# BAMresearch/PGDrome

Hardware: AMD Instinct MI355X
Metric: PGD fixed-point iters/sec + SpMV HBM GB/s, 256^3 P1 space x 1D param (higher is better)
Workload: dtype f64

## Files before the change

### include/pgd_amd.h

```cpp
#ifndef PGD_AMD_H
#define PGD_AMD_H

#include <stdint.h>

#ifdef __cplusplus
extern "C" {
#endif

typedef int64_t pgd_handle;

enum {
    PGD_OK = 0,
    PGD_ERR_INVALID = -1,
    PGD_ERR_HIP = -2,
    PGD_ERR_NOMEM = -3,
    PGD_ERR_LIMIT = -4,
    PGD_ERR_SINGULAR = -5,
    PGD_ERR_NODEVICE = -6,
    PGD_ERR_TIMEOUT = -7,
    PGD_ERR_PEER = -8
};

enum {
    PGD_ATOM_MASS = 0,
// ... 168 lines not shown
                   double threshold, double *sample_stats, pgd_handle env_min, pgd_handle env_max, pgd_handle exceed,
                   pgd_handle fields);

int pgd_cell_gradient(pgd_handle ctx, pgd_handle mesh, pgd_handle u, const double *L, int q, pgd_handle scale_or_0,
                      pgd_handle out);

int pgd_eval_batch_norm(pgd_handle ctx, const pgd_handle *modes, int k, int q, const double *coefs, int64_t s, int want,
                        double threshold, double *sample_stats, pgd_handle env_min, pgd_handle env_max, pgd_handle exceed,
                        pgd_handle fields);
int pgd_eval_batch_grad(pgd_handle ctx, pgd_handle mesh, const pgd_handle *modes, int k, const double *L, int q,
                        pgd_handle scale_or_0, const double *coefs, int64_t s, int want, double threshold, double *sample_stats,
                        pgd_handle env_min, pgd_handle env_max, pgd_handle exceed, pgd_handle fields);
int pgd_eval_norm_last_shape(pgd_handle ctx, int *rows, int *staged);

enum {
    PGD_TUNE_PCG_SCALAR_S = 56,
    PGD_TUNE_PCG_FOLD_MARCH = 55,
    PGD_TUNE_BLOCK_STORAGE = 54,
    PGD_TUNE_PCG_RECOMPUTE_Q = 53,
    PGD_TUNE_EVAL_SAMPLE_CHUNK = 52,
    PGD_TUNE_EVAL_GRID_MAX = 51,
    PGD_TUNE_EVAL_VARIANT = 50,
    PGD_TUNE_PUSH_IN_UPDATE = 49,
    PGD_TUNE_STENCIL_ROWS = 48,
    PGD_TUNE_DIA_MARCH3 = 47,
    PGD_TUNE_SHARD_ONE_MARCH = 46,
    PGD_TUNE_HALO_OVERLAP_MIN_ROWS = 45,
    PGD_TUNE_COMM_SELF_PERIODIC = 44,
    PGD_TUNE_PCG_DERIVE_SCALED = 43,
    PGD_TUNE_MG_MARCH_MIN = 42,
// ... 33 lines not shown
    PGD_TUNE_SPMV_VARIANT = 13,
    PGD_TUNE_SPMV_ZCHUNK = 6,
    PGD_TUNE_SPMV_SYM = 3,
    PGD_TUNE_SPMV_DICT = 2
};
int pgd_tune(pgd_handle ctx, int knob, int64_t value);

int pgd_prof_enable(pgd_handle ctx, int on);
int pgd_prof_read(pgd_handle ctx, int64_t *launches, double *seconds, double *alg_bytes);
int pgd_prof_read_own(pgd_handle ctx, double *own_bytes);
int pgd_prof_read_update(pgd_handle ctx, int64_t *launches, double *seconds, double *bytes);
int pgd_prof_read_dropped(pgd_handle ctx, int64_t *dropped);
int pgd_prof_event_overhead(pgd_handle ctx, double *seconds);
int pgd_kernel_counts(pgd_handle ctx, int64_t *out, int n);
int pgd_pcg_recompute_counts(pgd_handle ctx, int64_t *updates);
int pgd_classify_counts(pgd_handle ctx, int64_t *full, int64_t *cached);
int pgd_mg_counts(pgd_handle ctx, int64_t *solves, int64_t *fallbacks);
int pgd_vmg_counts(pgd_handle ctx, int64_t *solves, int64_t *fallbacks, int64_t *levels);
int pgd_vmg_times(pgd_handle ctx, double *setup_ms, int64_t *march_passes);
int pgd_cmg_counts(pgd_handle ctx, int64_t *solves, int64_t *fallbacks, int64_t *levels);
int pgd_cmg_times(pgd_handle ctx, double *setup_ms, int64_t *march_passes);
int pgd_mg_slab_setup(pgd_handle ctx, pgd_handle A, int nz_global, int z_first, int64_t own0, int64_t own1,
                      int64_t *n_coarse, int *applies);
int pgd_mg_slab_fix_start(pgd_handle ctx, pgd_handle A, pgd_handle b, pgd_handle x, int64_t own0, int64_t own1);
int pgd_mg_slab_down(pgd_handle ctx, pgd_handle r, pgd_handle t);
int pgd_mg_slab_restrict(pgd_handle ctx, pgd_handle t, pgd_handle b1);
int pgd_mg_coarse(pgd_handle ctx, pgd_handle b1, pgd_handle x1);
int pgd_mg_slab_up(pgd_handle ctx, pgd_handle r, pgd_handle x1, pgd_handle t, pgd_handle z, int slot, double *dot);
int pgd_calib_stream(pgd_handle ctx, pgd_handle vec, int bytes_per_lane, int store);
int pgd_timer_start(pgd_handle ctx);
// ... 7 lines not shown
```

### pgdrome_amd/_lib.py

```python
from __future__ import annotations

import ctypes as C
from pathlib import Path

import numpy as np

LIB_PATH = Path(__file__).resolve().parent / "lib" / "libpgd_amd.so"

H = C.c_int64
I64 = C.c_int64
I32 = C.c_int32
F64 = C.c_double
PD = C.POINTER(C.c_double)
PI32 = C.POINTER(C.c_int32)
PI64 = C.POINTER(C.c_int64)
PH = C.POINTER(C.c_int64)
VP = C.c_void_p

PU8 = C.POINTER(C.c_uint8)
HALO_FN = C.CFUNCTYPE(C.c_int, VP, H, I64, I64, I64, I64)
ALLREDUCE_FN = C.CFUNCTYPE(C.c_int, VP, C.c_int, C.c_int)

SIGNATURES = {
    "pgd_ctx_create": (C.c_int, [C.c_int, VP, PH]),
# ... 95 lines not shown
    "pgd_comm_push": (C.c_int, [H, C.c_int, C.POINTER(C.c_int)]),
    "pgd_comm_allreduce_attach": (C.c_int, [H, PU8, C.POINTER(C.c_int)]),
    "pgd_comm_allreduce_direct": (C.c_int, [H, C.c_int, C.POINTER(C.c_int)]),
    "pgd_pcg_solve_sharded": (C.c_int, [H, H, H, H, I64, I64, I64, I64, F64, F64, C.c_int, C.POINTER(C.c_int), PD]),
    "pgd_op_symmetrize": (C.c_int, [H, H, C.POINTER(C.c_int)]),
    "pgd_op_classify": (C.c_int, [H, H, C.POINTER(C.c_int)]),
    "pgd_tune": (C.c_int, [H, C.c_int, I64]),
    "pgd_prof_enable": (C.c_int, [H, C.c_int]),
    "pgd_prof_read": (C.c_int, [H, PI64, PD, PD]),
    "pgd_prof_read_own": (C.c_int, [H, PD]),
    "pgd_prof_read_update": (C.c_int, [H, PI64, PD, PD]),
    "pgd_prof_read_dropped": (C.c_int, [H, PI64]),
    "pgd_prof_event_overhead": (C.c_int, [H, PD]),
    "pgd_kernel_counts": (C.c_int, [H, PI64, C.c_int]),
    "pgd_pcg_recompute_counts": (C.c_int, [H, PI64]),
    "pgd_classify_counts": (C.c_int, [H, PI64, PI64]),
    "pgd_mg_counts": (C.c_int, [H, PI64, PI64]),
    "pgd_vmg_counts": (C.c_int, [H, PI64, PI64, PI64]),
    "pgd_vmg_times": (C.c_int, [H, C.POINTER(C.c_double), PI64]),
    "pgd_cmg_counts": (C.c_int, [H, PI64, PI64, PI64]),
    "pgd_cmg_times": (C.c_int, [H, C.POINTER(C.c_double), PI64]),
    "pgd_calib_stream": (C.c_int, [H, H, C.c_int, C.c_int]),
    "pgd_timer_start": (C.c_int, [H]),
    "pgd_timer_stop": (C.c_int, [H, PD]),
}

NSLOTS = 64
EVAL_STATS, EVAL_ENVELOPE, EVAL_EXCEED, EVAL_FIELDS = 1, 2, 4, 8
TUNE_EVAL_VARIANT, TUNE_EVAL_GRID_MAX, TUNE_EVAL_SAMPLE_CHUNK = 50, 51, 52
TUNE_BLOCK_STORAGE = 54
TUNE_PCG_FOLD_MARCH, TUNE_PCG_SCALAR_S = 55, 56
BLOCK_F32, BLOCK_F64, BLOCK_MAXK = 0, 1, 64


ERR_TIMEOUT, ERR_PEER = -7, -8


class PgdError(RuntimeError):
    def __init__(self, code, msg):
        super().__init__(f"libpgd_amd error {code}: {msg}")
        self.code = code


_lib = None


# ... 631 lines not shown
                    update_launches=un.value, update_seconds=us.value, update_bytes=ub.value, dropped_noop_samples=dr.value,
                    event_overhead=ov.value)

    KERNEL_FAMILIES = ("csr", "csr_dict", "sym_rows", "dia_rows", "dia_march", "multi", "diac_march", "stencil_march")

    def kernel_counts(self):
        out = (C.c_int64 * 8)()
        self._ck(self.lib.pgd_kernel_counts(self.h, out, 8))
        return {k: int(out[i]) for i, k in enumerate(self.KERNEL_FAMILIES)}

    def pcg_recompute_updates(self):
        n = I64()
        self._ck(self.lib.pgd_pcg_recompute_counts(self.h, C.byref(n)))
        return n.value

    def classify_counts(self):
        full, cached = I64(), I64()
        self._ck(self.lib.pgd_classify_counts(self.h, C.byref(full), C.byref(cached)))
        return {"full": full.value, "cached": cached.value}

    def precondition(self, multigrid):
        self.tune(40, 1 if multigrid else 0)
        return self.mg_stats()["solves"]

    def mg_stats(self):
        a, b = I64(), I64()
        self._ck(self.lib.pgd_mg_counts(self.h, C.byref(a), C.byref(b)))
        return {"solves": a.value, "fallbacks": b.value}

    def precondition_variable(self, on):
# ... 30 lines not shown
```

### pgdrome_amd/csrc/pgd_ctx.hip

```cpp
#include <algorithm>
#include <cstdarg>
#include <cstring>
#include <mutex>

#include "pgd_internal.h"

namespace pgd {

static std::mutex g_mu;
static std::vector<std::unique_ptr<Ctx>> g_ctx;
static std::string g_global_err;

Ctx *get_ctx(pgd_handle h) {
    std::lock_guard<std::mutex> lk(g_mu);
    if (h < 1 || h > (pgd_handle)g_ctx.size()) return nullptr;
    return g_ctx[h - 1].get();
}

int fail(Ctx *c, int code, const char *fmt, ...) {
    char buf[512];
    va_list ap;
    va_start(ap, fmt);
    vsnprintf(buf, sizeof buf, fmt, ap);
    va_end(ap);
// ... 424 lines not shown

int pgd_kernel_counts(pgd_handle h, int64_t *out, int n) {
    PGD_CTX(c, h);
    if (!out || n < 0) return fail(c, PGD_ERR_INVALID, "kernel_counts: invalid arguments");
    for (int k = 0; k < n; ++k) out[k] = k < 8 ? c->kcount[k] : 0;
    return PGD_OK;
}

int pgd_pcg_recompute_counts(pgd_handle h, int64_t *updates) {
    PGD_CTX(c, h);
    if (!updates) return fail(c, PGD_ERR_INVALID, "pcg_recompute_counts: invalid arguments");
    *updates = c->pcg_recompute_launches;
    return PGD_OK;
}

int pgd_timer_start(pgd_handle h) {
    PGD_CTX(c, h);
    for (auto &e : c->timer_ev)
        if (!e) PGD_HIP(c, hipEventCreate(&e));
    PGD_HIP(c, hipEventRecord(c->timer_ev[0], c->stream));
    return PGD_OK;
}

int pgd_timer_stop(pgd_handle h, double *seconds) {
    PGD_CTX(c, h);
    if (!c->timer_ev[0] || !c->timer_ev[1] || !seconds) return fail(c, PGD_ERR_INVALID, "timer_stop: no timer running");
    PGD_HIP(c, hipEventRecord(c->timer_ev[1], c->stream));
    PGD_HIP(c, hipEventSynchronize(c->timer_ev[1]));
    float ms = 0.f;
    PGD_HIP(c, hipEventElapsedTime(&ms, c->timer_ev[0], c->timer_ev[1]));
// ... 6 lines not shown
```

### pgdrome_amd/csrc/pgd_internal.h

```cpp
#pragma once

#include <hip/hip_runtime.h>

#include <chrono>
#include <cstdint>
#include <cstdio>
#include <map>
#include <memory>
#include <string>
#include <vector>

#include "../../include/pgd_amd.h"

namespace pgd {

constexpr int WAVE = 64;
constexpr int TPB = 256;
constexpr int MAX_VEC_BLOCKS = 2048;
constexpr int N_XCD = 8;
constexpr int DICT_MAXP = 256;
constexpr int DICT_DLEN = 32;
constexpr size_t PAD_BYTES = 256;

enum { S_PQ = 2, S_TOL2 = 5, S_DMIN = 7 , S_TMP = 8  };
// ... 191 lines not shown
    int num_cu = 256;
    int spmv_dict = 1;
    int spmv_rows = 64;
    int64_t spmv_grid_min_plane_bytes = 0;
    int spmv_zchunk_force = 0;
    int fault_iteration = -1;
    int fault_stage = 0;
    int fault_stall_ms = 0;
    int64_t pcg_small_ss_rows = (int64_t)1 << 22;
    int pcg_small_ss = 1;
    int pcg_stream_hints = 1;
    int pcg_lag_x = 1;
    int pcg_recompute_q = 1;
    int64_t pcg_recompute_launches = 0;
    int pcg_fold_march = 0;
    int pcg_scalar_s = 1;
    int asm_lattice = 1;
    int spmv_fetch_depth = 6;
    int spmv_zchunk_coded2 = 96;
    int spmv_zchunk_coded = 24;
    int pcg_exact_phase = 1;
    int pcg_fold_finish = 1;
    int atom_fast = 1;
    int lazy_csr = 1;
    uint64_t next_serial = 1;
    int pcg_precond = 0;
    struct Mg *mg = nullptr;
    struct Mg *mg_slab = nullptr;
    int64_t mg_solves = 0, mg_fallbacks = 0;
    struct Vmg *vmg = nullptr;
// ... 114 lines not shown
int vec_sqrt(Ctx *c, double *v, int64_t n);
int vec_div_mul(Ctx *c, double *x, const double *sc, int64_t n, int mul);
int ensure_vals(Ctx *c, const Mesh *m, Csr *a);
bool atom_fast_form(Ctx *c, const Mesh *m, Csr *a, int64_t r0, int64_t r1);
int dia_classify(Ctx *c, const Mesh *m, Csr *a, int zrange_lo = -1, int zrange_hi = -1);
bool stencil_row_range(const Ctx *c, const Mesh *m, const Csr *a, int64_t r0, int64_t r1);
bool stencil_whole_grid(const Ctx *c, const Mesh *m, const Csr *a);
struct StencilFold {
    const double *prod; int nprod;
    const double *vec_in; int nvec;
    int par;
};
int stencil_update_blocks(const Ctx *c, const Mesh *m);
int launch_stencil_update(Ctx *c, const Mesh *m, const Csr *a, const double *p_in, double *p_out, double *x, double *r, const double *s,
                          double *pairs, int lag, double s_free = 0.0, const StencilFold *fold = nullptr);
int launch_stencil_pass(Ctx *c, const uint8_t *cls, int ident, const double cst[8], int nx, int ny, int nz, int zm0, int zm1,
                        const double *x, const double *b, double *y, double w, int epi, bool dot, int *nparts, int z0 = 0, int z1 = -1);
bool mg_prepare(Ctx *c, const Mesh *m, const Csr *a);
int mg_fix_start(Ctx *c, const Csr *a, const double *b, double *x, int64_t n);
int mg_vcycle(Ctx *c, const double *r, bool dot, int *nparts, double *z_out = nullptr);
double *mg_result(Ctx *c);
void mg_release(Ctx *c);
struct Vmg;
bool vmg_prepare(Ctx *c, Vmg *&M, const Mesh *m, const Csr *a);
int vmg_fix_start(Ctx *c, Vmg *M, const double *sc, const double *b, double *x, int64_t n);
int vmg_vcycle(Ctx *c, Vmg *M, const double *r, bool dot, int *nparts, double *z_out, int64_t *marches);
double *vmg_result(Vmg *M);
void vmg_note_setup(Ctx *c);
void vmg_release(Ctx *c);
bool cmg_prepare(Ctx *c, const Mesh *m, const Mesh *base, const Csr *a);
// ... 113 lines not shown
```

### pgdrome_amd/csrc/pgd_pcg.hip

```cpp
#include "pgd_internal.h"

#include <cmath>

#include <cstring>

#include <algorithm>

namespace pgd {

constexpr int MAXT = 8;
constexpr int CHECK_EVERY = 16;
constexpr int PROF_EAGER_EVERY = 8;

struct CombineArgs {
    const double *in[MAXT];
    double coef[MAXT];
    int n;
};

__global__ __launch_bounds__(TPB) void k_combine(CombineArgs A, double *__restrict__ out, const int *__restrict__ cols,
                                                 const uint8_t *__restrict__ colmask, int64_t nnz) {
    for (int64_t k = (int64_t)blockIdx.x * TPB + threadIdx.x; k < nnz; k += (int64_t)gridDim.x * TPB) {
        double s = 0.0;
#pragma unroll
// ... 1244 lines not shown
}

struct PcgRun {
    static constexpr int S_INIT = 18, S_PAIR = 16;
    Ctx *c; const Mesh *m; Csr *o; const double *b; double *x; int64_t n;
    double *r, *z, *p, *q, *sc;
    double *part2 = nullptr, *part2b = nullptr;
    int gvec = 0, g2v = 0;
    PcgForm form = PGD_PCG_FORM_TEXTBOOK;
    PcgPrecond precond = PGD_PCG_PRECOND_JACOBI;
    bool scaled = false, lag_x = false;
    bool x_scaled = false;
    bool virt = false;
    double s_free = 0.0;
    bool fold_march = false;
    double st_saved[8] = {0, 0, 0, 0, 0, 0, 0, 0};
    ~PcgRun() {
        if (virt) {
            for (int s2 = 0; s2 < 8; ++s2) o->st_c[s2] = st_saved[s2];
            o->st_virtual = false;
        }
        if (!x_scaled) return;
        (void)vec_div_mul(c, x, sc, n, 1);
        if (!virt) invalidate_slots();
    }
    void invalidate_slots() { o->uvals_valid = false; o->uvals_scaled = false; }
    int out(int k) const { return S_PAIR + 2 * (k & 1); }
    int old(int k) const { return S_PAIR + 2 * ((k + 1) & 1); }
    int g2() const { return grid_for((n + 1) / 2); }
};
// ... 66 lines not shown
    PGD_TRY(pcg_precond_prepare(R));
    PGD_TRY(launch_spmv_op(c, R.m, R.o, R.x, R.q, nullptr, 0, n, false, true, nullptr, nullptr));
    const int g = grid_for(n);
    PGD_TRY(ensure_partials(c, 4 * (int64_t)MAX_VEC_BLOCKS));
    k_pcg_init_s<<<g, TPB, 0, c->stream>>>(R.b, R.q, R.sc, R.r, R.p, n, c->partials);
    PGD_LAUNCH_CHECK(c);
    return reduce_partials(c, c->partials, g, 3, R.S_INIT, -1, 0, 0);
}

static int pcg_setup_unscaled(PcgRun &R) {
    PGD_TRY(pcg_precond_prepare(R));
    PGD_TRY(launch_spmv_op(R.c, R.m, R.o, R.x, R.q, nullptr, 0, R.n, false, true, nullptr, nullptr));
    return pcg_init(R.c, R.b, R.q, R.o->dinv, R.r, R.z, R.p, 0, R.n, R.S_INIT);
}

static int pcg_choose_and_seed(PcgRun &R) {
    Ctx *c = R.c;
    const int64_t n = R.n;
    if (R.precond != PGD_PCG_PRECOND_JACOBI) {
        int np = 0;
        PGD_TRY(pcg_precond_apply(R, R.r, R.p, &np));
        PGD_TRY(reduce_partials(c, c->partials, np, 1, R.S_INIT, -1, 0, 0));
    }
    PGD_TRY(ensure_work(c, 6, 4 * (int64_t)MAX_VEC_BLOCKS));
    c->pcg_last_precond = R.precond;
    c->pcg_last_form = R.form = pcg_choose(c, R.precond, R.scaled, n, R.m->sym_nx > 0, stencil_whole_grid(c, R.m, R.o));
    R.lag_x = c->pcg_lag_x && pcg_single_sync(R.form);
    R.g2v = grid_for((n + 1) / 2, TPB, (n > ((int64_t)1 << 20) && n <= c->pcg_small_ss_rows && c->pcg_small_ss) ? 512 : MAX_VEC_BLOCKS);
    R.gvec = R.form == PGD_PCG_FORM_SINGLE_SYNC_RECOMPUTE ? stencil_update_blocks(c, R.m) : R.g2v;
    R.fold_march = R.form == PGD_PCG_FORM_SINGLE_SYNC_RECOMPUTE && c->pcg_fold_march;
    const int64_t half = 2 * std::max<int64_t>(MAX_VEC_BLOCKS, R.fold_march ? R.gvec : 0);
    PGD_TRY(ensure_work(c, 6, std::max<int64_t>(2 * half, 2 * (int64_t)R.gvec)));
    R.part2 = c->work[6];
    R.part2b = R.part2 + half;
    if (!pcg_single_sync(R.form)) return PGD_OK;
    const bool two = R.form == PGD_PCG_FORM_TWO_LAUNCH || R.fold_march;
    k_pcg1_seed<<<8, TPB, 0, c->stream>>>(two ? R.part2b : R.part2, R.gvec, c->slots, R.S_INIT, R.S_INIT + 1);
    if (two) PGD_HIP(c, hipMemsetAsync(c->slots + S1F_ALPHA, 0, 6 * sizeof(double), c->stream));
    PGD_LAUNCH_CHECK(c);
    return PGD_OK;
}

static int pcg_product(PcgRun &R, int *nparts, bool reduce = true) {
    PGD_TRY(launch_spmv_op(R.c, R.m, R.o, R.p, R.q, R.p, 0, R.n, true, true, R.c->flags, nparts));
    return reduce ? reduce_partials(R.c, R.c->partials, *nparts, 1, S_PQ, 0, 0, 0) : PGD_OK;
}
static int pcg_update_scaled(PcgRun &R, int k) {
    k_pcg_xr_s<<<R.g2(), TPB, 0, R.c->stream>>>(R.x, R.r, R.p, R.q, R.sc, R.n, R.c->slots, R.old(k), S_PQ, R.c->partials, R.c->flags);
    PGD_LAUNCH_CHECK(R.c);
    return reduce_partials(R.c, R.c->partials, R.g2(), 2, R.out(k), 2, R.out(k) + 1, S_TOL2);
}
static int pcg_update_unscaled(PcgRun &R, int k, double *z) {
    return pcg_xr(R.c, R.x, R.r, R.p, R.q, z ? R.o->dinv : nullptr, z, 0, R.n, R.old(k), S_PQ, R.out(k), 1, S_TOL2);
}
// ... 77 lines not shown
    return pcg1_end(R, I);
}

static int pcg_iter_single_sync(PcgRun &R, int k) {
    Pcg1Iter I;
    PGD_TRY(pcg1_begin(R, k, R.p, true, true, &I));
    launch_pcg1_update(R.c, R.g2v, R.x, R.r, R.p, R.q, R.sc, 0, R.n, S1_ALPHA, S1_BETA, R.part2, I.lag, 0, -1, nullptr);
    return pcg1_end(R, I);
}

static int pcg_iter_single_sync_recompute(PcgRun &R, int k) {
    Pcg1Iter I;
    const int par = k & 1;
    double *p_cur = par ? R.q : R.p, *p_next = par ? R.p : R.q;
    const double s_free = (R.virt && R.c->pcg_scalar_s) ? R.s_free : 0.0;
    PGD_TRY(pcg1_begin(R, k, p_cur, false, !R.fold_march, &I));
    if (R.fold_march) {
        const StencilFold F{I.prod, I.nparts, par ? R.part2 : R.part2b, R.gvec, par};
        PGD_TRY(launch_stencil_update(R.c, R.m, R.o, p_cur, p_next, R.x, R.r, R.sc, par ? R.part2b : R.part2, I.lag, s_free, &F));
    } else PGD_TRY(launch_stencil_update(R.c, R.m, R.o, p_cur, p_next, R.x, R.r, R.sc, R.part2, I.lag, s_free));
    return pcg1_end(R, I, 8.0);
}

static int pcg_enqueue(PcgRun &R, int start, int count) {
    for (int k = start; k < start + count; ++k) {
        R.c->prof_iter = k;
        switch (R.form) {
        case PGD_PCG_FORM_PRECOND: PGD_TRY(pcg_iter_precond(R, k)); break;
        case PGD_PCG_FORM_TEXTBOOK: PGD_TRY(pcg_iter_textbook(R, k)); break;
        case PGD_PCG_FORM_TWO_LAUNCH: PGD_TRY(pcg_iter_two_launch(R, k)); break;
        case PGD_PCG_FORM_FOLDED: PGD_TRY(pcg_iter_folded(R, k)); break;
        case PGD_PCG_FORM_SINGLE_SYNC: PGD_TRY(pcg_iter_single_sync(R, k)); break;
        case PGD_PCG_FORM_SINGLE_SYNC_RECOMPUTE: PGD_TRY(pcg_iter_single_sync_recompute(R, k)); break;
        case PGD_PCG_FORM_DEFERRED_X: PGD_TRY(pcg_iter_deferred_x(R, k)); break;
        case PGD_PCG_FORM_PLAIN: PGD_TRY(pcg_iter_plain(R, k)); break;
        }
    }
    return PGD_OK;
}

static int pcg_drive(PcgRun &R, int CE, int maxit, int f[4], int &enq, double *dbg) {
    Ctx *c = R.c;
    hipGraphExec_t gexec = nullptr;
    if (dbg) { (void)hipStreamSynchronize(c->stream); dbg[0] = host_now(); }
    if (maxit >= CE) {
        PGD_TRY(ensure_partials(c, std::max<int64_t>(4 * (int64_t)MAX_VEC_BLOCKS, 2 * ((R.n + 63) / 64) + 64)));
        PGD_TRY(ensure_work(c, 5, 4096));
        const bool prof_saved = c->prof;
        c->prof = false;
        hipGraph_t graph = nullptr;
        if (hipStreamBeginCapture(c->stream, hipStreamCaptureModeThreadLocal) == hipSuccess) {
            const int rc = pcg_enqueue(R, 0, CE);
            const hipError_t e = hipStreamEndCapture(c->stream, &graph);
            if (rc != PGD_OK || e != hipSuccess || !graph ||
                hipGraphInstantiate(&gexec, graph, nullptr, nullptr, 0) != hipSuccess)
                gexec = nullptr;
            if (graph) (void)hipGraphDestroy(graph);
            (void)hipGetLastError();
        }
        c->prof = prof_saved;
    }
// ... 42 lines not shown
    if (dbg) { (void)hipStreamSynchronize(c->stream); dbg[2] = host_now(); }
    if (gexec) (void)hipGraphExecDestroy(gexec);
    return rc_loop;
}

static int pcg_finish(PcgRun &R, const int f[4], int *iters, double *relres) {
    Ctx *c = R.c;
    if (R.scaled) {
        const int g = grid_for(R.n);
        R.x_scaled = false;
        const bool pending = R.form == PGD_PCG_FORM_DEFERRED_X && f[0] != 0 && f[1] > 0;
        const bool lag_pending = R.lag_x && f[1] > 0 && ((f[1] - 1) & 1) == 0;
        const int last_par = f[1] > 0 ? (f[1] - 1) & 1 : 0;
        const bool two = R.form == PGD_PCG_FORM_TWO_LAUNCH || R.fold_march;
        const double *p_live = R.form == PGD_PCG_FORM_SINGLE_SYNC_RECOMPUTE && (f[1] & 1) ? R.q : R.p;
        k_scale_out<<<g, TPB, 0, c->stream>>>(R.x, R.r, R.sc, R.n, c->partials, (pending || lag_pending) ? p_live : nullptr, c->slots,
                                              R.S_PAIR + 2 * (f[1] & 1), S_PQ, lag_pending ? 1 : 0,
                                              two ? S1F_ALPHA + last_par : S1_ALPHA, two ? S1F_BETA + last_par : S1_BETA);
        PGD_LAUNCH_CHECK(c);
        PGD_TRY(reduce_partials(c, c->partials, g, 1, S_TMP, -1, 0, 0));
        if (!R.virt) R.invalidate_slots();
    }
    PGD_LAUNCH_CHECK(c);
    double s[PGD_NSLOTS];
    PGD_HIP(c, hipMemcpyAsync(s, c->slots, sizeof s, hipMemcpyDeviceToHost, c->stream));
    PGD_HIP(c, hipStreamSynchronize(c->stream));
    if (R.precond == PGD_PCG_PRECOND_VMG) vmg_note_setup(c);
    if (R.precond == PGD_PCG_PRECOND_CMG) cmg_note_setup(c);
    if (iters) *iters = f[1];
    const double rr = R.scaled ? s[S_TMP] : (f[1] > 0) ? s[R.S_PAIR + 2 * ((f[1] - 1) & 1) + 1] : s[R.S_INIT + 1];
    const double bb = s[R.S_INIT + 2];
// ... 290 lines not shown
```

### pgdrome_amd/csrc/pgd_spmv.hip

```cpp
#include <chrono>
#include <cstring>

#include "pgd_internal.h"
#include "pgd_dia_march.h"

#include <algorithm>

namespace pgd {

constexpr int SPMV_CAP = 4096;
constexpr int SPMV_VROUNDS = 8;
constexpr int SPMV_CROUNDS = 4;
constexpr int MAXY = 8;

struct SpmvArgs {
    const int *row_ptr, *cols;
    const double *vals, *x, *w;
    double *y, *partials;
    const int *flags;
    int row_begin, row_end;
};

typedef double d2_t __attribute__((ext_vector_type(2)));
typedef int i4_t __attribute__((ext_vector_type(4)));
// ... 1358 lines not shown
        }
    }
    if (EPI == 3 && !u_exact) dot2 = dot;
    if (DOT) {
        for (int pass = 0; pass < (A.qq ? 2 : 1); ++pass) {
            const double sum = wave_sum(pass ? dot2 : dot);
            __syncthreads();
            if (lane == 0) s_red[wv] = sum;
            __syncthreads();
            if (tid == 0) A.partials[A.qq ? 2 * b + pass : b] = (s_red[0] + s_red[1]) + (s_red[2] + s_red[3]);
        }
    }
}
#undef PGD_ST_STAMP
#undef PGD_ST_WHATIF

struct StencilInfo { int ok, ident, base, split; double c[8]; int zm0, zm1, g_lo, g_hi; };

__global__ void k_stencil_pick(const uint8_t *__restrict__ cls, double *__restrict__ table, const int *__restrict__ info,
                               int nx, int ny, int z_lo, int z_hi, StencilInfo *S) {
    if (threadIdx.x != 0 || blockIdx.x != 0) return;
    S->ok = 0; S->ident = -1; S->base = -1; S->split = 0;
    const int ncls = info[0];
    if (info[1] != 0 || ncls <= 0 || ncls >= CLS_MAX || z_hi <= z_lo) return;
    const int64_t mid = (int64_t)nx * ny * ((z_lo + z_hi) / 2) + (int64_t)nx * (ny / 2) + nx / 2;
    for (int k = 0; k < ncls; ++k) {
        bool id = table[k * 8 + cls_pos(0)] == 1.0;
        for (int s = 1; s < 8; ++s) id = id && table[k * 8 + cls_pos(s)] == 0.0;
        if (id) S->ident = k;
    }
// ... 1032 lines not shown
    if (fold) {
        F.fold_prod = fold->prod; F.fold_nprod = fold->nprod; F.fold_vec = fold->vec_in; F.fold_nvec = fold->nvec;
        F.fold_par = fold->par & 1; F.fold_flags = c->flags;
    }
    const bool nt = c->pcg_stream_hints != 0;
    if (sh.rows_per_thread == 2) {
        if (nt) k_spmv_stencil_march<true, true, 3, true, 2, 3, 2><<<sh.wgs, 256, 0, c->stream>>>(F);
        else k_spmv_stencil_march<true, true, 3, false, 2, 3, 2><<<sh.wgs, 256, 0, c->stream>>>(F);
    } else if (nt) k_spmv_stencil_march<true, true, 3, true, 2, 3><<<sh.wgs, 256, 0, c->stream>>>(F);
    else k_spmv_stencil_march<true, true, 3, false, 2, 3><<<sh.wgs, 256, 0, c->stream>>>(F);
    c->pcg_recompute_launches += 1;
    PGD_LAUNCH_CHECK(c);
    return PGD_OK;
}

constexpr int GRAM_MAXV = 17;
struct MultiDotArgs {
    const double *w, *b;
    const double *v[GRAM_MAXV];
    int nv;
    int64_t lo, hi;
    double *partials;
};

__global__ __launch_bounds__(TPB) void k_multidot(MultiDotArgs A) {
    __shared__ double s_red[4];
    double acc[GRAM_MAXV + 1];
#pragma unroll
    for (int m = 0; m <= GRAM_MAXV; ++m) acc[m] = 0.0;
    for (int64_t i = A.lo + (int64_t)blockIdx.x * TPB + threadIdx.x; i < A.hi; i += (int64_t)gridDim.x * TPB) {
// ... 194 lines not shown
    if (knob == PGD_TUNE_PCG_DERIVE_SCALED && value >= 0 && value <= 1) { c->pcg_derive_scaled = (int)value; return PGD_OK; }
    if (knob == PGD_TUNE_COMM_SELF_PERIODIC && value >= 0 && value <= 1) { c->comm.self_periodic = value != 0; return PGD_OK; }
    if (knob == PGD_TUNE_HALO_OVERLAP_MIN_ROWS && value >= 0) { c->comm.overlap_min_rows = value; return PGD_OK; }
    if (knob == PGD_TUNE_SHARD_ONE_MARCH && value >= 0 && value <= 1) { c->shard_one_march = (int)value; return PGD_OK; }
    if (knob == PGD_TUNE_DIA_MARCH3 && value >= 0 && value <= 1) { c->dia_march3 = (int)value; return PGD_OK; }
    if (knob == PGD_TUNE_STENCIL_ROWS && (value == 0 || value == 2 || value == 4)) { c->stencil_rows = (int)value; return PGD_OK; }
    if (knob == PGD_TUNE_PUSH_IN_UPDATE && (value == 0 || value == 1)) { c->push_in_update = (int)value; return PGD_OK; }
    if (knob == PGD_TUNE_MG_CHUNK && value >= 2 && value <= 16 && value % 2 == 0) { c->mg_chunk = (int)value; return PGD_OK; }
    if (knob == PGD_TUNE_MG_MARCH_MIN && value >= 0 && value <= 1 << 20) { c->mg_march_min = (int)value; return PGD_OK; }
    if (knob == PGD_TUNE_EVAL_VARIANT && value >= 0 && value <= 1) { c->eval_variant = (int)value; return PGD_OK; }
    if (knob == PGD_TUNE_EVAL_GRID_MAX && value >= 0 && value <= 1 << 20) { c->eval_grid_max = (int)value; return PGD_OK; }
    if (knob == PGD_TUNE_EVAL_SAMPLE_CHUNK && value >= 0 && value <= 1024) { c->eval_chunk = (int)value; return PGD_OK; }
    if (knob == PGD_TUNE_PCG_RECOMPUTE_Q && value >= 0 && value <= 1) { c->pcg_recompute_q = (int)value; return PGD_OK; }
    if (knob == PGD_TUNE_PCG_FOLD_MARCH && value >= 0 && value <= 1) { c->pcg_fold_march = (int)value; return PGD_OK; }
    if (knob == PGD_TUNE_PCG_SCALAR_S && value >= 0 && value <= 1) { c->pcg_scalar_s = (int)value; return PGD_OK; }
    if (knob == PGD_TUNE_BLOCK_STORAGE && value >= 0 && value <= 2) { c->block_storage = (int)value; return PGD_OK; }
    return fail(c, PGD_ERR_INVALID, "tune: unknown knob %d or value out of range", knob);
}

int pgd_spmv(pgd_handle h, pgd_handle ah, pgd_handle xh, pgd_handle yh, int64_t r0, int64_t r1) {
    PGD_CTX(c, h);
    Csr *a = get_csr(c, ah);
    Mesh *m = a ? get_mesh(c, a->mesh) : nullptr;
    Vec *x = get_vec(c, xh), *y = get_vec(c, yh);
    if (!a || !m || !x || !y || x->n != m->nv || y->n != m->nv || x == y)
        return fail(c, PGD_ERR_INVALID, "spmv: invalid handles, size mismatch or x aliases y");
    if (atom_fast_form(c, m, a, r0, r1)) return launch_spmv_op(c, m, a, x->d, y->d, nullptr, r0, r1, false, true, nullptr, nullptr);
    if (c->spmv_sym && c->atom_fast && m->sym_nx > 0 && !a->immutable && a->uvals && a->uvals_valid && !a->uvals_scaled && !a->st_virtual) {
        const int64_t plane = (int64_t)m->sym_nx * m->sym_ny;
        const int64_t q0 = r0 < 0 ? 0 : r0, q1 = r1 < 0 ? m->nv : r1;
// ... 260 lines not shown
```

Measured before the change: 18.17.

## Fuse PCG vector update and stencil product into a single z-march kernel

Adds a fused stencil march kernel that applies the PCG update (x, r, p), stages the new search direction in shared memory, and computes the next operator product A·p and its dot partials in the same pass over z. The r vector is double-buffered and the first product is seeded before iterations begin. The aim is to avoid a separate product launch and a second full read of p per iteration, cutting HBM traffic. The cost is more shared memory and halo recompute per tile, and the path is tied to specific stencil shapes. It is enabled by default.

```diff
diff --git a/include/pgd_amd.h b/include/pgd_amd.h
--- a/include/pgd_amd.h
+++ b/include/pgd_amd.h
@@ -206,6 +206,7 @@
 int pgd_eval_norm_last_shape(pgd_handle ctx, int *rows, int *staged);
 
 enum {
+    PGD_TUNE_PCG_FUSED_MARCH = 57,
     PGD_TUNE_PCG_SCALAR_S = 56,
     PGD_TUNE_PCG_FOLD_MARCH = 55,
     PGD_TUNE_BLOCK_STORAGE = 54,
@@ -269,6 +270,7 @@
 int pgd_prof_event_overhead(pgd_handle ctx, double *seconds);
 int pgd_kernel_counts(pgd_handle ctx, int64_t *out, int n);
 int pgd_pcg_recompute_counts(pgd_handle ctx, int64_t *updates);
+int pgd_pcg_fused_counts(pgd_handle ctx, int64_t *marches);
 int pgd_classify_counts(pgd_handle ctx, int64_t *full, int64_t *cached);
 int pgd_mg_counts(pgd_handle ctx, int64_t *solves, int64_t *fallbacks);
 int pgd_vmg_counts(pgd_handle ctx, int64_t *solves, int64_t *fallbacks, int64_t *levels);
diff --git a/pgdrome_amd/_lib.py b/pgdrome_amd/_lib.py
--- a/pgdrome_amd/_lib.py
+++ b/pgdrome_amd/_lib.py
@@ -133,6 +133,7 @@
     "pgd_prof_event_overhead": (C.c_int, [H, PD]),
     "pgd_kernel_counts": (C.c_int, [H, PI64, C.c_int]),
     "pgd_pcg_recompute_counts": (C.c_int, [H, PI64]),
+    "pgd_pcg_fused_counts": (C.c_int, [H, PI64]),
     "pgd_classify_counts": (C.c_int, [H, PI64, PI64]),
     "pgd_mg_counts": (C.c_int, [H, PI64, PI64]),
     "pgd_vmg_counts": (C.c_int, [H, PI64, PI64, PI64]),
@@ -148,7 +149,7 @@
 EVAL_STATS, EVAL_ENVELOPE, EVAL_EXCEED, EVAL_FIELDS = 1, 2, 4, 8
 TUNE_EVAL_VARIANT, TUNE_EVAL_GRID_MAX, TUNE_EVAL_SAMPLE_CHUNK = 50, 51, 52
 TUNE_BLOCK_STORAGE = 54
-TUNE_PCG_FOLD_MARCH, TUNE_PCG_SCALAR_S = 55, 56
+TUNE_PCG_FOLD_MARCH, TUNE_PCG_SCALAR_S, TUNE_PCG_FUSED_MARCH = 55, 56, 57
 BLOCK_F32, BLOCK_F64, BLOCK_MAXK = 0, 1, 64
 
 
@@ -810,6 +811,11 @@
         self._ck(self.lib.pgd_pcg_recompute_counts(self.h, C.byref(n)))
         return n.value
 
+    def pcg_fused_marches(self):
+        n = I64()
+        self._ck(self.lib.pgd_pcg_fused_counts(self.h, C.byref(n)))
+        return n.value
+
     def classify_counts(self):
         full, cached = I64(), I64()
         self._ck(self.lib.pgd_classify_counts(self.h, C.byref(full), C.byref(cached)))
diff --git a/pgdrome_amd/csrc/pgd_ctx.hip b/pgdrome_amd/csrc/pgd_ctx.hip
--- a/pgdrome_amd/csrc/pgd_ctx.hip
+++ b/pgdrome_amd/csrc/pgd_ctx.hip
@@ -462,6 +462,13 @@
     return PGD_OK;
 }
 
+int pgd_pcg_fused_counts(pgd_handle h, int64_t *marches) {
+    PGD_CTX(c, h);
+    if (!marches) return fail(c, PGD_ERR_INVALID, "pcg_fused_counts: invalid arguments");
+    *marches = c->pcg_fused_launches;
+    return PGD_OK;
+}
+
 int pgd_timer_start(pgd_handle h) {
     PGD_CTX(c, h);
     for (auto &e : c->timer_ev)
diff --git a/pgdrome_amd/csrc/pgd_internal.h b/pgdrome_amd/csrc/pgd_internal.h
--- a/pgdrome_amd/csrc/pgd_internal.h
+++ b/pgdrome_amd/csrc/pgd_internal.h
@@ -229,6 +229,8 @@
     int pcg_recompute_q = 1;
     int64_t pcg_recompute_launches = 0;
     int pcg_fold_march = 0;
+    int64_t pcg_fused_launches = 0;
+    int pcg_fused_march = 1;
     int pcg_scalar_s = 1;
     int asm_lattice = 1;
     int spmv_fetch_depth = 6;
@@ -373,6 +375,9 @@
 int stencil_update_blocks(const Ctx *c, const Mesh *m);
 int launch_stencil_update(Ctx *c, const Mesh *m, const Csr *a, const double *p_in, double *p_out, double *x, double *r, const double *s,
                           double *pairs, int lag, double s_free = 0.0, const StencilFold *fold = nullptr);
+bool stencil_fused_ok(const Ctx *c, const Mesh *m, const Csr *a);
+int launch_stencil_fused(Ctx *c, const Mesh *m, const Csr *a, const double *p_in, double *p_out, double *x, const double *r_in, double *r_out,
+                         const double *s, double *pairs, int lag, double s_free);
 int launch_stencil_pass(Ctx *c, const uint8_t *cls, int ident, const double cst[8], int nx, int ny, int nz, int zm0, int zm1,
                         const double *x, const double *b, double *y, double w, int epi, bool dot, int *nparts, int z0 = 0, int z1 = -1);
 bool mg_prepare(Ctx *c, const Mesh *m, const Csr *a);
diff --git a/pgdrome_amd/csrc/pgd_pcg.hip b/pgdrome_amd/csrc/pgd_pcg.hip
--- a/pgdrome_amd/csrc/pgd_pcg.hip
+++ b/pgdrome_amd/csrc/pgd_pcg.hip
@@ -1282,6 +1282,10 @@
     bool virt = false;
     double s_free = 0.0;
     bool fold_march = false;
+    bool fused = false;
+    double *r2 = nullptr;
+    const double *fprod = nullptr;
+    int fnprod = 0;
     double st_saved[8] = {0, 0, 0, 0, 0, 0, 0, 0};
     ~PcgRun() {
         if (virt) {
@@ -1378,6 +1382,8 @@
     return pcg_init(R.c, R.b, R.q, R.o->dinv, R.r, R.z, R.p, 0, R.n, R.S_INIT);
 }
 
+static int64_t pcg_partials_needed(int64_t n) { return std::max<int64_t>(4 * (int64_t)MAX_VEC_BLOCKS, 2 * ((n + 63) / 64) + 64); }
+
 static int pcg_choose_and_seed(PcgRun &R) {
     Ctx *c = R.c;
     const int64_t n = R.n;
@@ -1392,7 +1398,8 @@
     R.lag_x = c->pcg_lag_x && pcg_single_sync(R.form);
     R.g2v = grid_for((n + 1) / 2, TPB, (n > ((int64_t)1 << 20) && n <= c->pcg_small_ss_rows && c->pcg_small_ss) ? 512 : MAX_VEC_BLOCKS);
     R.gvec = R.form == PGD_PCG_FORM_SINGLE_SYNC_RECOMPUTE ? stencil_update_blocks(c, R.m) : R.g2v;
-    R.fold_march = R.form == PGD_PCG_FORM_SINGLE_SYNC_RECOMPUTE && c->pcg_fold_march;
+    R.fused = R.form == PGD_PCG_FORM_SINGLE_SYNC_RECOMPUTE && c->pcg_fused_march && stencil_fused_ok(c, R.m, R.o);
+    R.fold_march = R.form == PGD_PCG_FORM_SINGLE_SYNC_RECOMPUTE && c->pcg_fold_march && !R.fused;
     const int64_t half = 2 * std::max<int64_t>(MAX_VEC_BLOCKS, R.fold_march ? R.gvec : 0);
     PGD_TRY(ensure_work(c, 6, std::max<int64_t>(2 * half, 2 * (int64_t)R.gvec)));
     R.part2 = c->work[6];
@@ -1402,6 +1409,20 @@
     k_pcg1_seed<<<8, TPB, 0, c->stream>>>(two ? R.part2b : R.part2, R.gvec, c->slots, R.S_INIT, R.S_INIT + 1);
     if (two) PGD_HIP(c, hipMemsetAsync(c->slots + S1F_ALPHA, 0, 6 * sizeof(double), c->stream));
     PGD_LAUNCH_CHECK(c);
+    if (R.fused) {
+        PGD_TRY(ensure_work(c, 4, n));
+        R.r2 = c->work[4];
+        PGD_TRY(ensure_partials(c, pcg_partials_needed(n)));
+        PGD_TRY(ensure_work(c, 5, 4096));
+        if (c->prof) c->prof_seen &= ~(int64_t)3;
+        c->spmv_qq = 1;
+        const int rc = launch_spmv_op(c, R.m, R.o, R.p, R.q, R.p, 0, n, true, false, c->flags, &R.fnprod);
+        c->spmv_qq = 0;
+        PGD_TRY(rc);
+        if (R.fnprod != R.gvec) return fail(c, PGD_ERR_INVALID, "pcg_solve: the product's launch is not the update's");
+        c->kcount[KC_STENCIL_MARCH] -= 1;
+        PGD_TRY(stage_product_partials(c, &R.fprod, &R.fnprod));
+    }
     return PGD_OK;
 }
 
@@ -1509,6 +1530,17 @@
     const int par = k & 1;
     double *p_cur = par ? R.q : R.p, *p_next = par ? R.p : R.q;
     const double s_free = (R.virt && R.c->pcg_scalar_s) ? R.s_free : 0.0;
+    if (R.fused) {
+        Ctx *c = R.c;
+        I.lag = R.lag_x ? 1 + (k & 1) : 0;
+        if (R.gvec <= 8192 && R.fprod != c->partials) return fail(c, PGD_ERR_INVALID, "pcg_solve: the partial sums moved under the fused march");
+        k_pcg1_scalars<<<1, 1024, 0, c->stream>>>(R.fprod, R.fnprod, R.part2, R.gvec, c->slots, c->flags);
+        PGD_TRY(update_timing_begin(c, &I.timed));
+        PGD_TRY(launch_stencil_fused(c, R.m, R.o, p_cur, p_next, R.x, par ? R.r2 : R.r, par ? R.r : R.r2, R.sc, R.part2, I.lag, s_free));
+        PGD_TRY(pcg1_end(R, I, 8.0));
+        I.nparts = R.gvec;
+        return stage_product_partials(c, &I.prod, &I.nparts);
+    }
     PGD_TRY(pcg1_begin(R, k, p_cur, false, !R.fold_march, &I));
     if (R.fold_march) {
         const StencilFold F{I.prod, I.nparts, par ? R.part2 : R.part2b, R.gvec, par};
@@ -1539,7 +1571,7 @@
     hipGraphExec_t gexec = nullptr;
     if (dbg) { (void)hipStreamSynchronize(c->stream); dbg[0] = host_now(); }
     if (maxit >= CE) {
-        PGD_TRY(ensure_partials(c, std::max<int64_t>(4 * (int64_t)MAX_VEC_BLOCKS, 2 * ((R.n + 63) / 64) + 64)));
+        PGD_TRY(ensure_partials(c, pcg_partials_needed(R.n)));
         PGD_TRY(ensure_work(c, 5, 4096));
         const bool prof_saved = c->prof;
         c->prof = false;
@@ -1612,7 +1644,8 @@
         const int last_par = f[1] > 0 ? (f[1] - 1) & 1 : 0;
         const bool two = R.form == PGD_PCG_FORM_TWO_LAUNCH || R.fold_march;
         const double *p_live = R.form == PGD_PCG_FORM_SINGLE_SYNC_RECOMPUTE && (f[1] & 1) ? R.q : R.p;
-        k_scale_out<<<g, TPB, 0, c->stream>>>(R.x, R.r, R.sc, R.n, c->partials, (pending || lag_pending) ? p_live : nullptr, c->slots,
+        const double *r_live = R.fused && (f[1] & 1) ? R.r2 : R.r;
+        k_scale_out<<<g, TPB, 0, c->stream>>>(R.x, r_live, R.sc, R.n, c->partials, (pending || lag_pending) ? p_live : nullptr, c->slots,
                                               R.S_PAIR + 2 * (f[1] & 1), S_PQ, lag_pending ? 1 : 0,
                                               two ? S1F_ALPHA + last_par : S1_ALPHA, two ? S1F_BETA + last_par : S1_BETA);
         PGD_LAUNCH_CHECK(c);
diff --git a/pgdrome_amd/csrc/pgd_spmv.hip b/pgdrome_amd/csrc/pgd_spmv.hip
--- a/pgdrome_amd/csrc/pgd_spmv.hip
+++ b/pgdrome_amd/csrc/pgd_spmv.hip
@@ -1396,6 +1396,291 @@
 }
 #undef PGD_ST_STAMP
 #undef PGD_ST_WHATIF
+
+struct FusedArgs : StencilArgs {
+    double *ur_out = nullptr;
+    double *prod_pairs = nullptr;
+};
+
+template <int RW, int W>
+__device__ __forceinline__ void stencil_chain_rows(const double *xm, const double *xc, const double *xp, const double (&c)[8], double (&acc)[RW]) {
+    double M[RW + 1][2], C[RW + 2][3], Q[RW + 1][2];
+#pragma unroll
+    for (int j = 0; j <= RW; ++j) { M[j][0] = xm[(j - 1) * W - 1]; M[j][1] = xm[(j - 1) * W]; }
+#pragma unroll
+    for (int j = 0; j <= RW + 1; ++j) {
+        if (j <= RW) C[j][0] = xc[(j - 1) * W - 1];
+        C[j][1] = xc[(j - 1) * W];
+        if (j >= 1) C[j][2] = xc[(j - 1) * W + 1];
+    }
+#pragma unroll
+    for (int j = 0; j <= RW; ++j) { Q[j][0] = xp[j * W]; Q[j][1] = xp[j * W + 1]; }
+    __builtin_amdgcn_sched_barrier(0);
+#pragma unroll
+    for (int r = 0; r < RW; ++r) acc[r] = c[7] * M[r][0];
+#define PGD_ST_ROWS(cc, V)                           \
+    _Pragma("unroll") for (int r = 0; r < RW; ++r) acc[r] = fma(cc, V, acc[r])
+    PGD_ST_ROWS(c[6], M[r][1]);
+    PGD_ST_ROWS(c[5], M[r + 1][0]);
+    PGD_ST_ROWS(c[4], M[r + 1][1]);
+    PGD_ST_ROWS(c[3], C[r][0]);
+    PGD_ST_ROWS(c[2], C[r][1]);
+    PGD_ST_ROWS(c[1], C[r + 1][0]);
+    PGD_ST_ROWS(c[0], C[r + 1][1]);
+    PGD_ST_ROWS(c[1], C[r + 1][2]);
+    PGD_ST_ROWS(c[2], C[r + 2][1]);
+    PGD_ST_ROWS(c[3], C[r + 2][2]);
+    PGD_ST_ROWS(c[4], Q[r][0]);
+    PGD_ST_ROWS(c[5], Q[r][1]);
+    PGD_ST_ROWS(c[6], Q[r + 1][0]);
+    PGD_ST_ROWS(c[7], Q[r + 1][1]);
+#undef PGD_ST_ROWS
+}
+
+template <bool NTY, int RWT>
+__global__ __launch_bounds__(256, 2) void k_pcg1_fused_march(FusedArgs A) {
+    static_assert(RWT == 4 || RWT == 2, "rows per thread");
+    constexpr int NT = 256, RW = RWT, PY = 4 * RW;
+    constexpr int W2 = DM_HX + 2, H2 = PY + 4, SLOT2 = W2 * H2;
+    constexpr int W1 = DM_HX, H1 = PY + 2, SLOT1 = W1 * H1;
+    constexpr int NH2 = SLOT2 - 64 * PY;
+    constexpr int NR1 = SLOT1 - 64 * PY;
+    constexpr int NQ = RW + 2;
+    constexpr int OOB = (int)0x40000000;
+    constexpr int AUX_RX = NTY ? 2 : 0;
+    static_assert(NH2 <= 2 * NT && NR1 <= NT, "halo cells per thread");
+    static_assert((4 * SLOT2 + 4 * SLOT1 + 4) * 8 <= 80 * 1024, "two workgroups per CU");
+    __shared__ double s_p[4 * SLOT2];
+    __shared__ double s_n[4 * SLOT1];
+    __shared__ double s_red[4];
+    if (A.flags && A.flags[0]) return;
+    const double u_alpha = A.slots[S1_ALPHA], u_beta = A.slots[S1_BETA];
+    const bool u_exact = A.flags[3] != 0;
+    const bool u_skip_x = A.lag == 1 && u_beta >= LAG_MIN_BETA;
+    const bool u_two = A.lag == 2 && A.slots[S1_PEND] != 0.0;
+    const double u_alpha_p = u_two ? A.slots[S1_ALPHA_PREV] : 0.0;
+    const double u_ibeta_p = u_two ? 1.0 / A.slots[S1_BETA_PREV] : 0.0;
+    const bool u_s_known = A.s_free > 0.0;
+    if (A.lag == 1 && blockIdx.x == 0 && threadIdx.x == 0) A.slots[S1_PEND] = u_skip_x ? 1.0 : 0.0;
+    const int tid = threadIdx.x, lane = tid & 63, wv = tid >> 6;
+    const int b = xcd_remap(blockIdx.x, gridDim.x);
+    const int per_chunk = A.tiles_x * A.tiles_y;
+    const int chunk = b / per_chunk, tile = b - chunk * per_chunk;
+    const int ty = tile / A.tiles_x, tx = tile - ty * A.tiles_x;
+    const int x0 = tx * 64, y0 = ty * PY;
+    const int64_t P = (int64_t)A.nx * A.ny;
+    const unsigned P8 = (unsigned)(P * 8);
+    const int centre2 = (RW * wv + 2) * W2 + lane + 2;
+    const int centre1 = (RW * wv + 1) * W1 + lane + 1;
+    const int za = A.z0 + chunk * A.zchunk, zb = min(A.z1, za + A.zchunk);
+    if (za >= zb) {
+        if (tid == 0) { A.partials[2 * b] = 0.0; A.partials[2 * b + 1] = 0.0; A.prod_pairs[2 * b] = 0.0; A.prod_pairs[2 * b + 1] = 0.0; }
+        return;
+    }
+    int lv[NQ], sv[RW], hc[2];
+    double m[RW];
+    bool fixr[RW];
+    unsigned fix = 0;
+    int ring_c2 = centre2, ring_c1 = 0, ring_off = OOB;
+    {
+        const uint8_t *cz = A.cls + P * min(max(A.zm0, 0), A.nz - 1);
+        auto code = [&](int gx, int gy, bool *in, bool *masked) {
+            *in = gx >= 0 && gx < A.nx && gy >= 0 && gy < A.ny;
+            const int off = *in ? gx + A.nx * gy : 0;
+            *masked = *in && A.ident >= 0 && (int)cz[off] == A.ident;
+            return off;
+        };
+#pragma unroll
+        for (int q = 0; q < RW; ++q) {
+            bool in, masked;
+            const int off = code(x0 + lane, y0 + RW * wv + q, &in, &masked);
+            lv[q] = in ? 8 * off : OOB;
+            sv[q] = lv[q];
+            m[q] = (in && !masked) ? 1.0 : 0.0;
+            fixr[q] = in && masked;
+            if (fixr[q]) fix |= 1u << q;
+        }
+#pragma unroll
+        for (int j = 0; j < 2; ++j) {
+            const int k = tid + j * NT;
+            int lx, ly;
+            if (k < 2 * W2) { ly = k / W2; lx = k - ly * W2; }
+            else if (k < 4 * W2) { ly = (k - 2 * W2) / W2; lx = k - 2 * W2 - ly * W2; ly += PY + 2; }
+            else { const int k2 = k - 4 * W2, cx = k2 & 3; ly = 2 + (k2 >> 2); lx = cx < 2 ? cx : 64 + cx; }
+            bool in, masked;
+            const int off = code(x0 - 2 + lx, y0 - 2 + ly, &in, &masked);
+            const bool have = k < NH2;
+            lv[RW + j] = (have && in && !masked) ? 8 * off : OOB;
+            hc[j] = have ? ly * W2 + lx : -1;
+        }
+        if (tid < NR1) {
+            int lx, ly;
+            if (tid < W1) { lx = tid; ly = 0; }
+            else if (tid < 2 * W1) { lx = tid - W1; ly = H1 - 1; }
+            else if (tid < 2 * W1 + PY) { lx = 0; ly = tid - 2 * W1 + 1; }
+            else { lx = W1 - 1; ly = tid - 2 * W1 - PY + 1; }
+            bool in, masked;
+            const int off = code(x0 - 1 + lx, y0 - 1 + ly, &in, &masked);
+            ring_c1 = ly * W1 + lx;
+            ring_c2 = (ly + 1) * W2 + lx + 1;
+            ring_off = (in && !masked) ? 8 * off : OOB;
+        }
+    }
+    const bool ring_on = ring_off != OOB;
+    const double cc[8] = {A.c[0], A.c[1], A.c[2], A.c[3], A.c[4], A.c[5], A.c[6], A.c[7]};
+    double dot = 0.0, dot2 = 0.0;
+    double pdot = 0.0, pdot2 = 0.0;
+    auto rsrc_of = [&](const double *plane_ptr, bool live) {
+        return __builtin_amdgcn_make_buffer_rsrc(const_cast<double *>(plane_ptr), 0, live ? (int)P8 : 0, 0x00020000);
+    };
+    auto ld = [&](auto r, int off, int aux) -> double {
+        return aux ? __builtin_bit_cast(double, __builtin_amdgcn_raw_buffer_load_b64(r, off, 0, AUX_RX))
+                   : __builtin_bit_cast(double, __builtin_amdgcn_raw_buffer_load_b64(r, off, 0, 0));
+    };
+    const int zd0 = min(A.zv0, A.zs0), zd1 = max(A.zv1, A.zs1);
+    auto fetch = [&](int zz, double (&v)[NQ]) {
+        const auto r = rsrc_of(A.x + P * (int64_t)zz, zz >= zd0 && zz < zd1 && zz <= zb + 1);
+#pragma unroll
+        for (int q = 0; q < NQ; ++q) v[q] = ld(r, lv[q], 0);
+    };
+    auto stage = [&](int zz, const double (&v)[NQ], double (&own)[RW]) {
+        double *dst = s_p + (zz & 3) * SLOT2;
+        const bool data = zz >= A.zs0 && zz < A.zs1;
+#pragma unroll
+        for (int q = 0; q < RW; ++q) { dst[centre2 + q * W2] = data ? v[q] * m[q] : 0.0; own[q] = v[q]; }
+#pragma unroll
+        for (int j = 0; j < 2; ++j)
+            if (hc[j] >= 0) dst[hc[j]] = data ? v[RW + j] : 0.0;
+    };
+    auto update = [&](int z, const double (&xo)[RW], double (&pn)[RW]) {
+        const bool own_plane = z >= za && z < zb;
+        const bool main = z >= A.zm0 && z < A.zm1, verified = z >= A.zv0 && z < A.zv1;
+        const bool data = z >= A.zs0 && z < A.zs1;
+        double *dn = s_n + (z & 3) * SLOT1;
+        if (!(main || (verified && own_plane))) {
+#pragma unroll
+            for (int r = 0; r < RW; ++r) { dn[centre1 + r * W1] = 0.0; pn[r] = 0.0; }
+            if (tid < NR1) dn[ring_c1] = 0.0;
+            return;
+        }
+        const int64_t oz = P * (int64_t)z;
+        const auto dr = rsrc_of(A.ur + oz, true);
+        const auto dx = rsrc_of(A.ux + oz, own_plane && !u_skip_x);
+        double ur[RW], ux[RW], us[RW], rring;
+#pragma unroll
+        for (int r = 0; r < RW; ++r) ur[r] = ld(dr, sv[r], 1);
+        rring = ld(dr, main ? ring_off : OOB, 0);
+#pragma unroll
+        for (int r = 0; r < RW; ++r) ux[r] = ld(dx, sv[r], 1);
+        if (!u_s_known) {
+            const auto ds = rsrc_of(A.us + oz, own_plane && u_exact);
+#pragma unroll
+            for (int r = 0; r < RW; ++r) us[r] = ld(ds, sv[r], 0);
+        }
+        double qv[RW], qring = 0.0, pring = 0.0;
+        if (main) {
+            const double *xm = s_p + ((z - 1) & 3) * SLOT2, *xc = s_p + (z & 3) * SLOT2, *xp = s_p + ((z + 1) & 3) * SLOT2;
+            double acc[RW];
+            stencil_chain_rows<RW, W2>(xm + centre2, xc + centre2, xp + centre2, cc, acc);
+            if (tid < NR1) {
+                double accr[1];
+                stencil_chain_rows<1, W2>(xm + ring_c2, xc + ring_c2, xp + ring_c2, cc, accr);
+                qring = accr[0];
+                pring = xc[ring_c2];
+            }
+#pragma unroll
+            for (int r = 0; r < RW; ++r) qv[r] = fixr[r] ? xo[r] : acc[r];
+        } else {
+#pragma unroll
+            for (int r = 0; r < RW; ++r) qv[r] = xo[r];
+        }
+        const unsigned ones = main ? fix : ~0u;
+        const auto so_r = rsrc_of(A.ur_out + oz, own_plane), so_p = rsrc_of(A.y + oz, own_plane);
+#pragma unroll
+        for (int r = 0; r < RW; ++r) {
+            const double pi = xo[r], r0 = ur[r];
+            if (own_plane && !u_skip_x) {
+                double xi = ux[r];
+                if (u_two) xi = fma(u_alpha_p, (pi - r0) * u_ibeta_p, xi);
+                xi = fma(u_alpha, pi, xi);
+                __builtin_amdgcn_raw_buffer_store_b64(__builtin_bit_cast(st_v2i, xi), dx, sv[r], 0, AUX_RX);
+            }
+            const double ri = fma(-u_alpha, qv[r], r0);
+            const double pv = fma(u_beta, pi, ri);
+            __builtin_amdgcn_raw_buffer_store_b64(__builtin_bit_cast(st_v2i, ri), so_r, sv[r], 0, AUX_RX);
+            __builtin_amdgcn_raw_buffer_store_b64(__builtin_bit_cast(st_v2i, pv), so_p, sv[r], 0, 0);
+            const bool in = sv[r] != OOB;
+            pn[r] = in ? pv : 0.0;
+            if (own_plane) {
+                const double t = in ? ri : 0.0;
+                dot = fma(t, t, dot);
+                if (u_exact) {
+                    const double sr = u_s_known ? (((ones >> r) & 1u) ? 1.0 : A.s_free) : us[r];
+                    const double ts = t / (in ? sr : 1.0);
+                    dot2 = fma(ts, ts, dot2);
+                }
+            }
+            dn[centre1 + r * W1] = data ? pn[r] * m[r] : 0.0;
+        }
+        if (tid < NR1) {
+            const double ri = fma(-u_alpha, qring, rring);
+            const double pv = fma(u_beta, pring, ri);
+            dn[ring_c1] = (data && ring_on) ? pv : 0.0;
+        }
+    };
+    auto product = [&](int z, const double (&xo)[RW]) {
+        if (z >= A.zm0 && z < A.zm1) {
+            const double *xm = s_n + ((z - 1) & 3) * SLOT1 + centre1, *xc = s_n + (z & 3) * SLOT1 + centre1, *xp = s_n + ((z + 1) & 3) * SLOT1 + centre1;
+            double acc[RW];
+            stencil_chain_rows<RW, W1>(xm, xc, xp, cc, acc);
+#pragma unroll
+            for (int r = 0; r < RW; ++r) {
+                const double yv = fixr[r] ? xo[r] : acc[r];
+                pdot = fma(yv, xo[r], pdot);
+                const double t = sv[r] != OOB ? yv : 0.0;
+                pdot2 = fma(t, t, pdot2);
+            }
+        } else if (z >= A.zv0 && z < A.zv1) {
+#pragma unroll
+            for (int r = 0; r < RW; ++r) { pdot = fma(xo[r], xo[r], pdot); pdot2 = fma(xo[r], xo[r], pdot2); }
+        }
+    };
+    double rr[3][NQ];
+    double own[3][RW];
+    double pnew[3][RW];
+    {
+        double t0[NQ], t1[NQ], t2[NQ];
+        fetch(za - 2, t0); fetch(za - 1, t1); fetch(za, t2);
+#pragma unroll
+        for (int s = 0; s < 3; ++s) fetch(za + 1 + s, rr[s]);
+        stage(za - 2, t0, own[2]); stage(za - 1, t1, own[0]); stage(za, t2, own[1]);
+    }
+#pragma unroll
+    for (int s = 0; s < 3; ++s)
+#pragma unroll
+        for (int r = 0; r < RW; ++r) pnew[s][r] = 0.0;
+    __syncthreads();
+#pragma clang loop unroll(disable)
+    for (int z = za - 1; z <= zb + 1; z += 3) {
+#pragma unroll
+        for (int s = 0; s < 3; ++s) {
+            const int zs = z + s;
+            if (zs - 2 >= za && zs - 2 < zb) product(zs - 2, pnew[(s + 1) % 3]);
+            if (zs <= zb) update(zs, own[s], pnew[s]);
+            if (zs + 2 <= zb + 1) stage(zs + 2, rr[s], own[(s + 2) % 3]);
+            if (zs + 5 <= zb + 1) fetch(zs + 5, rr[s]);
+            lds_barrier();
+        }
+    }
+    if (!u_exact) dot2 = dot;
+    for (int pass = 0; pass < 4; ++pass) {
+        const double sum = wave_sum(pass == 0 ? dot : pass == 1 ? dot2 : pass == 2 ? pdot : pdot2);
+        __syncthreads();
+        if (lane == 0) s_red[wv] = sum;
+        __syncthreads();
+        if (tid == 0) (pass < 2 ? A.partials : A.prod_pairs)[2 * b + (pass & 1)] = (s_red[0] + s_red[1]) + (s_red[2] + s_red[3]);
+    }
+}
 
 struct StencilInfo { int ok, ident, base, split; double c[8]; int zm0, zm1, g_lo, g_hi; };
 
@@ -2458,6 +2743,48 @@
     return PGD_OK;
 }
 
+bool stencil_fused_ok(const Ctx *c, const Mesh *m, const Csr *a) {
+    if (!stencil_whole_grid(c, m, a) || a->st_g_lo || a->st_g_hi) return false;
+    const int64_t plane = (int64_t)m->sym_nx * m->sym_ny;
+    const int nz = (int)(m->nv / plane);
+    const StencilShape su = stencil_shape(c, m->sym_nx, m->sym_ny, nz, 3), sp = stencil_shape(c, m->sym_nx, m->sym_ny, nz, c->stencil_depth > 0 ? c->stencil_depth : 3);
+    return su.wgs == sp.wgs && su.zchunk == sp.zchunk && su.rows_per_thread == sp.rows_per_thread && su.tiles_y == sp.tiles_y &&
+           (sp.rows_per_thread == 4 || c->stencil_depth != 6);
+}
+
+int launch_stencil_fused(Ctx *c, const Mesh *m, const Csr *a, const double *p_in, double *p_out, double *x, const double *r_in, double *r_out,
+                         const double *s, double *pairs, int lag, double s_free) {
+    if (!stencil_fused_ok(c, m, a) || !c->flags || p_in == p_out || r_in == r_out)
+        return fail(c, PGD_ERR_INVALID, "fused march: the operator's products do not run in the stencil march over the whole grid");
+    const int64_t plane = (int64_t)m->sym_nx * m->sym_ny;
+    const int nz = (int)(m->nv / plane);
+    const StencilShape sh = stencil_shape(c, m->sym_nx, m->sym_ny, nz, 3);
+    PGD_TRY(ensure_partials(c, std::max<int64_t>(c->partials_off + 2 * (int64_t)sh.wgs, 4 * MAX_VEC_BLOCKS)));
+    FusedArgs F;
+    F.cls = a->cls; F.ident = a->st_ident; F.x = p_in; F.y = p_out; F.flags = c->flags;
+    F.zv0 = a->st_z0; F.zv1 = a->st_z1; F.zm0 = a->st_zm0; F.zm1 = a->st_zm1;
+    F.zs0 = a->st_zm0; F.zs1 = a->st_zm1;
+    for (int s2 = 0; s2 < 8; ++s2) F.c[s2] = a->st_c[s2];
+    F.nx = m->sym_nx; F.ny = m->sym_ny; F.nz = nz; F.z0 = 0; F.z1 = nz;
+    F.tiles_x = sh.tiles_x; F.tiles_y = sh.tiles_y; F.zchunk = sh.zchunk;
+    F.qq = 1; F.whatif = 0; F.b = nullptr; F.w = 0.0;
+    F.partials = pairs;
+    F.prod_pairs = c->partials + c->partials_off;
+    F.ur = const_cast<double *>(r_in); F.ur_out = r_out; F.ux = x; F.us = s; F.slots = c->slots; F.lag = lag;
+    F.s_free = s_free;
+    const bool nt = c->pcg_stream_hints != 0;
+    if (sh.rows_per_thread == 2) {
+        if (nt) k_pcg1_fused_march<true, 2><<<sh.wgs, 256, 0, c->stream>>>(F);
+        else k_pcg1_fused_march<false, 2><<<sh.wgs, 256, 0, c->stream>>>(F);
+    } else if (nt) k_pcg1_fused_march<true, 4><<<sh.wgs, 256, 0, c->stream>>>(F);
+    else k_pcg1_fused_march<false, 4><<<sh.wgs, 256, 0, c->stream>>>(F);
+    c->pcg_recompute_launches += 1;
+    c->pcg_fused_launches += 1;
+    c->kcount[KC_STENCIL_MARCH] += 1;
+    PGD_LAUNCH_CHECK(c);
+    return PGD_OK;
+}
+
 constexpr int GRAM_MAXV = 17;
 struct MultiDotArgs {
     const double *w, *b;
@@ -2682,6 +3009,7 @@
     if (knob == PGD_TUNE_PCG_RECOMPUTE_Q && value >= 0 && value <= 1) { c->pcg_recompute_q = (int)value; return PGD_OK; }
     if (knob == PGD_TUNE_PCG_FOLD_MARCH && value >= 0 && value <= 1) { c->pcg_fold_march = (int)value; return PGD_OK; }
     if (knob == PGD_TUNE_PCG_SCALAR_S && value >= 0 && value <= 1) { c->pcg_scalar_s = (int)value; return PGD_OK; }
+    if (knob == PGD_TUNE_PCG_FUSED_MARCH && value >= 0 && value <= 1) { c->pcg_fused_march = (int)value; return PGD_OK; }
     if (knob == PGD_TUNE_BLOCK_STORAGE && value >= 0 && value <= 2) { c->block_storage = (int)value; return PGD_OK; }
     return fail(c, PGD_ERR_INVALID, "tune: unknown knob %d or value out of range", knob);
 }
```

Result: faster. 19.36, median of 6 (+6.6%).
